# saikumar955078/rl-k8s-scheduler

Measured on AMD Instinct MI355X. Metric: env-steps/sec (node), batched rollout+policy update, 1/2/4/8 GPUs; %HBM BW, higher is better.
Workload: dtype fp32 (split-fp16 MFMA, fp32-accurate); 1 GPU; c4: 131,072 envs/GPU (1,048,576 over 8 GPUs) x 2-cloud table, T=128 rollout + GAE + PPO update (10 epochs x 256 minibatches of 65,536 rows/GPU, FCNet [256,256] tanh); envs_per_gpu=131072, rollout_steps=128, minibatch_per_gpu=65536, epochs=10, global_batch=16777216, global_envs=131072, global_minibatch=65536, sgd_precision=sf16, parallelism=dp1

## Files before the change

include/rlks.h:

```cpp
#ifndef RLKS_H
#define RLKS_H

#include <stdint.h>

#include "rlks_types.h"

#ifdef __cplusplus
extern "C" {
#endif

#define RLKS_OK 0
#define RLKS_ERR_ARG (-1)
#define RLKS_ERR_HIP (-2)
#define RLKS_ERR_UNSUPPORTED (-3)
#define RLKS_ERR_STATE (-4)

const char* rlks_last_error(void);
const char* rlks_version(void);

int rlks_debug_checks(unsigned long long* out);

typedef struct rlks_env rlks_env;

int rlks_env_create(const rlks_env_cfg* cfg, const double* cost_host, const double* lat_host,
// ... 48 lines not shown
             float lam, int T, int N, float* adv_dev, float* vtarg_dev, double* partials_dev,
             void* stream);
int rlks_gae_partials_count(int N);
int rlks_adv_stats(const double* partials_dev, int n_partials, double count, double* sums_dev,
                   void* stream);
int rlks_adv_finalize(const double* sums_dev, float* dyn_dev, void* stream);

#define RLKS_N_TENSORS 12
int rlks_mlp_layout(const rlks_mlp_desc* desc, int64_t* offsets12, int64_t* padded_count,
                    int64_t* real_count);

int rlks_policy_forward(const rlks_mlp_desc* desc, const float* params_dev, const float* obs_dev,
                        int n, float* logits_dev, float* values_dev, void* stream);

typedef struct rlks_rollout_bufs {
  float* obs;
  float* logits;
  float* values;
  int32_t* actions;
  float* logp;
  float* rewards;
  uint8_t* dones;
  float* adv;
  float* vtarg;
  int32_t T;
  int32_t N;
  int32_t global_lanes;
} rlks_rollout_bufs;

int rlks_rollout(rlks_env* env, const rlks_mlp_desc* desc, const float* params_dev,
                 const rlks_rollout_bufs* bufs, int explore, void* stream);
int rlks_policy_forward_ws(const rlks_mlp_desc* desc, const float* params_dev, const float* obs_dev, int n,
                           float* logits_dev, float* values_dev, void* workspace, int64_t ws_bytes, void* stream);
int rlks_gemm_sf16(const rlks_gemm_desc* desc, void* stream);
int rlks_absmax(const float* x, int rows, int cols, int ld, uint32_t* slot, void* stream);
int rlks_rollout_ws(rlks_env* env, const rlks_mlp_desc* desc, const float* params_dev,
                    const rlks_rollout_bufs* bufs, int explore, void* workspace, int64_t ws_bytes,
                    void* stream);

int rlks_minibatch_stride(const rlks_mlp_desc* desc);
int rlks_ppo_gather(const rlks_mlp_desc* desc, const rlks_rollout_bufs* bufs, uint64_t perm_seed,
                    int epoch, int64_t row0, int rows, const float* dyn_dev, float* mb_dev,
                    void* stream);
int rlks_ppo_gather_grouped(const rlks_mlp_desc* desc, const rlks_rollout_bufs* bufs, uint64_t perm_seed,
                            int epoch, int groups, int group0, int64_t row0, int rows, const float* dyn_dev,
                            float* mb_dev, void* stream);
int rlks_packed_stride(const rlks_mlp_desc* desc);
int rlks_ppo_pack(const rlks_mlp_desc* desc, const rlks_rollout_bufs* bufs, float* packed_dev, void* stream);
int rlks_ppo_gather_packed(const rlks_mlp_desc* desc, const float* packed_dev, int T, int N, uint64_t perm_seed,
                           int epoch, int groups, int group0, int64_t row0, int rows, float* mb_dev, void* stream);

int rlks_ppo_workspace_bytes(const rlks_mlp_desc* desc, int rows, int64_t* bytes);
int rlks_debug_sf_handoff(const rlks_mlp_desc* desc, int rows, void* workspace_dev, void** out);
int rlks_debug_wide_bufs(const rlks_mlp_desc* desc, int rows, void* workspace_dev, void** out);
int rlks_ppo_grad(const rlks_mlp_desc* desc, const rlks_ppo_coeffs* coeffs, const float* params_dev,
                  const float* dyn_dev, const float* mb_dev, int rows, float* grad_dev,
                  double* stats_dev, void* workspace_dev, int64_t workspace_bytes, void* stream);

#define RLKS_PHASE_FWD 1
#define RLKS_PHASE_DW2 2
#define RLKS_PHASE_DH1 4
#define RLKS_PHASE_REDUCE 8
#define RLKS_PHASE_ALL 15
#define RLKS_PHASE_FWD_PI 16
#define RLKS_PHASE_FWD_VF 32
#define RLKS_PHASE_PREP 64
#define RLKS_PHASE_F1A 128
#define RLKS_PHASE_F1B 256
int rlks_ppo_grad_phases(const rlks_mlp_desc* desc, const rlks_ppo_coeffs* coeffs, const float* params_dev,
                         const float* dyn_dev, const float* mb_dev, int rows, float* grad_dev, double* stats_dev,
                         void* workspace_dev, int64_t workspace_bytes, int phases, void* stream);

int rlks_ppo_grad_profile(const rlks_mlp_desc* desc, const rlks_ppo_coeffs* coeffs, const float* params_dev,
                          const float* dyn_dev, const float* mb_dev, int rows, float* grad_dev, double* stats_dev,
                          void* workspace_dev, int64_t workspace_bytes, int reps, double* ms_out, void* stream);

int rlks_sf_f1_fused(const rlks_mlp_desc* desc);

int rlks_adam_step(float* params_dev, const float* grad_dev, float* m_dev, float* v_dev, int64_t n,
                   float lr, float beta1, float beta2, float eps, int step, void* stream);
int rlks_ppo_sgd_step(const rlks_mlp_desc* desc, const rlks_ppo_coeffs* coeffs, float* params_dev,
                      const float* dyn_dev, const float* mb_dev, int rows, float* grad_dev, double* stats_dev,
                      float* adam_m_dev, float* adam_v_dev, int64_t n_params, float lr, float beta1, float beta2,
                      float eps, int step, int prev_fused, void* workspace, int64_t ws_bytes, void* stream);

typedef struct rlks_gather_next {
  const float* packed_dev;
  float* mb_dev;
  uint64_t perm_seed;
  int64_t row0;
  int T, N, epoch, groups, group0, rows;
} rlks_gather_next;
int rlks_ppo_sgd_step_next(const rlks_mlp_desc* desc, const rlks_ppo_coeffs* coeffs, float* params_dev,
                           const float* dyn_dev, const float* mb_dev, int rows, float* grad_dev, double* stats_dev,
                           float* adam_m_dev, float* adam_v_dev, int64_t n_params, float lr, float beta1, float beta2,
                           float eps, int step, int prev_fused, const rlks_gather_next* next, void* workspace,
                           int64_t ws_bytes, void* stream);

int rlks_ppo_grad_step(const rlks_mlp_desc* desc, const rlks_ppo_coeffs* coeffs, const float* params_dev,
                       const float* dyn_dev, const float* mb_dev, int rows, float* grad_dev, double* stats_dev,
                       int step, int prev_fused, void* workspace, int64_t ws_bytes, void* stream);
int rlks_ppo_grad_step_next(const rlks_mlp_desc* desc, const rlks_ppo_coeffs* coeffs, const float* params_dev,
                            const float* dyn_dev, const float* mb_dev, int rows, float* grad_dev, double* stats_dev,
                            int step, int prev_fused, const rlks_gather_next* next, void* workspace,
                            int64_t ws_bytes, void* stream);
int rlks_ppo_grad_step_part(const rlks_mlp_desc* desc, const rlks_ppo_coeffs* coeffs, const float* params_dev,
// ... 45 lines not shown
```

rl-k8s-scheduler_amd/csrc/ppo.hip:

```cpp
#include <cmath>

#include "sgd_sf16.h"
#include "wide_mlp.h"

namespace rlks {


struct RedTask {
  const float* part;
  float* out;
  double* out64;
  int64_t pstride;
  int P, len, G, V;
  int blk0;
  int mslot;
  int mbase;
  int kq;
};
constexpr int MAX_TASKS = 20;
struct AdamCo {
  float w1, b2, omb2, step_size, bc2_sqrt, eps;
};
__device__ __forceinline__ float adam_elem(float* __restrict__ p, float* __restrict__ m, float* __restrict__ v,
                                           int64_t i, float gi, const AdamCo& c) {
// ... 904 lines not shown
    RLKS_REQUIRE(bytes && rows > 0 && rows % 256 == 0, RLKS_ERR_ARG,
                 "rlks_ppo_workspace_bytes: split-fp16 rows must be a positive multiple of 256");
    *bytes = sf_ws_layout(d->obs_dim, d->n_actions, rows, nullptr).bytes;
    return RLKS_OK;
  }
  RLKS_REQUIRE(bytes && rows > 0 && rows % GB == 0, RLKS_ERR_ARG,
               "rlks_ppo_workspace_bytes: rows must be a positive multiple of 128");
  *bytes = ws_layout(d->obs_dim, d->n_actions, rows, nullptr).bytes;
  return RLKS_OK;
}

static int nrm_ws_at(const rlks_mlp_desc* d, int rows, void* workspace, int64_t ws_bytes, NrmWs& n) {
  int64_t gb = 0;
  if (int rc = grad_ws_bytes(d, rows, &gb)) return rc;
  gb = (gb + 255) / 256 * 256;
  n = nrm_ws(d, (char*)workspace + gb);
  RLKS_REQUIRE(ws_bytes >= gb + n.bytes, RLKS_ERR_ARG, "grad_clip: workspace too small (rlks_ppo_workspace_bytes)");
  return RLKS_OK;
}

}

extern "C" {

int rlks_ppo_workspace_bytes(const rlks_mlp_desc* d, int rows, int64_t* bytes) {
  if (int rc = grad_ws_bytes(d, rows, bytes)) return rc;
  *bytes = (*bytes + 255) / 256 * 256 + nrm_ws(d, nullptr).bytes;
  return RLKS_OK;
}

int rlks_grad_global_norm(const rlks_mlp_desc* d, const float* grad, int64_t n_params, double* norm_dev,
                          void* workspace, int64_t ws_bytes, void* stream) {
  if (int rc = check_desc(d)) return rc;
  RLKS_REQUIRE(grad && norm_dev && workspace, RLKS_ERR_ARG, "rlks_grad_global_norm: null argument");
  RLKS_REQUIRE(n_params == make_layout(d->obs_dim, d->hidden, d->n_actions).padded, RLKS_ERR_ARG,
               "rlks_grad_global_norm: n_params must be the padded layout size");
  const NrmWs n = nrm_ws(d, (char*)workspace);
  RLKS_REQUIRE(ws_bytes >= n.bytes, RLKS_ERR_ARG, "rlks_grad_global_norm: workspace too small");
  return norm_pass(d, grad, n, 1.f, norm_dev, nullptr, (hipStream_t)stream);
}

int rlks_debug_sf_handoff(const rlks_mlp_desc* d, int rows, void* ws, void** out) {
  if (int rc = check_desc(d)) return rc;
  RLKS_REQUIRE(out && ws && rows > 0 && rows % 256 == 0 && is_sf(d) && !is_wide(d),
               RLKS_ERR_ARG, "rlks_debug_sf_handoff: split-fp16 descriptor, rows % 256 == 0");
  const SfWs w = sf_ws_layout(d->obs_dim, d->n_actions, rows, (char*)ws);
  for (int net = 0; net < 2; ++net) {
    out[net] = w.n[net].dz2s;
    out[2 + net] = w.n[net].tile_edz;
  }
  return RLKS_OK;
}

int rlks_debug_wide_bufs(const rlks_mlp_desc* d, int rows, void* ws, void** out) {
  if (int rc = check_desc(d)) return rc;
  RLKS_REQUIRE(out && ws && rows > 0 && is_wide(d), RLKS_ERR_ARG, "rlks_debug_wide_bufs: wide descriptor");
  const WideWs w = wide_ws_layout(d->obs_dim, d->hidden, d->n_actions, rows, (char*)ws);
  for (int net = 0; net < 2; ++net) {
    out[3 * net] = w.n[net].h2;
    out[3 * net + 1] = w.n[net].out;
    out[3 * net + 2] = w.n[net].dout;
  }
  return RLKS_OK;
}

struct FusedAdam {
  float *p, *m, *v;
  AdamCo co;
  int step, prev_fused;
  bool apply = true;
  int64_t n = 0;
  float clip = 0.f;
};

static int sf_grad(const rlks_mlp_desc* d, const rlks_ppo_coeffs* co, const float* params, const float* dyn,
                   const float* mb, int M, float* grad, double* stats, void* workspace, int64_t ws_bytes, int phases,
                   hipStream_t s, const FusedAdam* fa = nullptr, const NextGather* nx = nullptr, int part = 0,
                   const NrmWs* nrm = nullptr, float clip = 0.f) {
  RLKS_REQUIRE(M > 0 && M % 256 == 0, RLKS_ERR_ARG, "rlks_ppo_grad: split-fp16 rows must be a positive multiple of 256");
  const int D = d->obs_dim, A = d->n_actions, H = HID;
  const SfWs w = sf_ws_layout(D, A, M, (char*)workspace);
  RLKS_REQUIRE(ws_bytes >= w.bytes, RLKS_ERR_ARG, "rlks_ppo_grad: workspace too small");
  const Layout L = make_layout(D, H, A);
  const bool f_pi = phases & (RLKS_PHASE_FWD | RLKS_PHASE_FWD_PI), f_vf = phases & (RLKS_PHASE_FWD | RLKS_PHASE_FWD_VF);
  if (part == 2) phases &= ~(RLKS_PHASE_PREP | RLKS_PHASE_DW2);
  if ((phases & (RLKS_PHASE_FWD | RLKS_PHASE_PREP)) && part != 2) {
    const int parity = fa ? ((fa->step - 1) & 1) : 0;
    if (int rc = sf_prep(d, w, params, s, false, parity, fa && fa->prev_fused, fa ? (unsigned)fa->step : 0u))
      return rc;
  }
  SfArgs a{};
  a.x = mb; a.x_stride = mb_stride(D, A); a.M = M; a.D = D; a.A_pi = A;
  a.tiles_per_split = w.tiles_per_split; a.co = *co; a.dyn = dyn; a.xsp = w.xsp;
  a.products = d->precision == RLKS_PRECISION_F16 ? 1 : 3;
  for (int net = 0; net < 2; ++net) {
    a.n[net] = w.n[net];
    const NetPtrs P = net_ptrs_host(params, L, net);
    a.n[net].b2 = P.b2; a.n[net].w3 = P.w3; a.n[net].b3 = P.b3;
  }
  const int f1ab = phases & (RLKS_PHASE_F1A | RLKS_PHASE_F1B);
  SfF1Form f1;
  if (part != 0) f1 = part == 1 ? SF_F1_A : SF_F1_B;
  else if (f1ab && !(f_pi || f_vf)) f1 = SfF1Form((f1ab & RLKS_PHASE_F1A ? SF_F1_A : 0) | (f1ab & RLKS_PHASE_F1B ? SF_F1_B : 0));
  else f1 = sf_f1_fused(A) ? SF_F1_FUSED : SF_F1_SPLIT;
  if (f_pi || f_vf) {
    if (int rc = launch_sf_f1(a, f_pi ? 0 : 1, (f_pi && f_vf) ? 2 : 1, A, s, f1)) return rc;
// ... 562 lines not shown
```

rl-k8s-scheduler_amd/csrc/sgd_sf16.hip:

```cpp
#include <cmath>
#include <type_traits>

#include "sgd_sf16.h"

namespace rlks {


using h8 = __attribute__((ext_vector_type(8))) _Float16;
using h4 = __attribute__((ext_vector_type(4))) _Float16;
using v4u = __attribute__((ext_vector_type(4))) unsigned;

constexpr int SF_ROWS = 256;
constexpr float SF_H1_SCALE = 16384.f;

__device__ __forceinline__ int sf_perm(int s, int h, int j) { return 16 * s + 8 * (j >> 2) + 4 * h + (j & 3); }
__device__ __forceinline__ int p16(int p) { return 16 * ((p >> 2) & 1) + 4 * (p >> 3) + (p & 3); }

__device__ __forceinline__ f32x16 mma(h8 a, h8 b, f32x16 c) {
  return __builtin_amdgcn_mfma_f32_32x32x16_f16(a, b, c, 0, 0, 0);
}
__device__ __forceinline__ f32x16 mma3(h8 ah, h8 al, h8 bh, h8 bl, f32x16 c) {
  c = mma(al, bh, c);
  c = mma(ah, bl, c);
  return mma(ah, bh, c);
}
template <int P>
__device__ __forceinline__ f32x16 mmaP(h8 ah, h8 al, h8 bh, h8 bl, f32x16 c) {
  if constexpr (P == 1) return __builtin_amdgcn_mfma_f32_32x32x16_f16(ah, bh, c, 0, 0, 0);
  else return mma3(ah, al, bh, bl, c);
}

__device__ __forceinline__ void split1(float x, _Float16& hi, _Float16& lo) {
  hi = (_Float16)x;
  lo = (_Float16)(x - (float)hi);
}
typedef _Float16 hf2 __attribute__((ext_vector_type(2)));
__device__ __forceinline__ void split2(float x0, float x1, unsigned& hi, unsigned& lo) {
  const hf2 h = {(_Float16)x0, (_Float16)x1};
  hi = __builtin_bit_cast(unsigned, h);
  unsigned l;
  asm("v_fma_mixlo_f16 %0, %1, 1.0, -%2 op_sel_hi:[0,0,1]\n\t"
      "v_fma_mixhi_f16 %0, %3, 1.0, -%2 op_sel:[0,0,1] op_sel_hi:[0,0,1]"
      : "=&v"(l)
      : "v"(x0), "v"(hi), "v"(x1));
  lo = l;
}
__device__ __forceinline__ void split8v(const float (&x)[8], h8& hi, h8& lo) {
  v4u h, l;
#pragma unroll
  for (int q = 0; q < 4; ++q) {
    unsigned a, b;
    split2(x[2 * q], x[2 * q + 1], a, b);
    h[q] = a;
    l[q] = b;
// ... 901 lines not shown
        float sum = 0.f;
        const int dq = (d & ~15) + 4 * (((d >> 2) & 3) ^ ((kk >> 1) & 3)) + (d & 3);
#pragma unroll
        for (int ww = 0; ww < W; ++ww) sum += sEp[jj * SLOT + (ww * 16 + kk) * 16 * DT + dq];
        if (d < ND - 1) N.part_w1[((size_t)blk * HID + k) * (ND - 1) + d] = sum;
        else N.part_b1[(size_t)blk * HID + k] = sum;
      }
      if (kt < 15) __syncthreads();
    }
  }
  FB_STAMP(5);
}

template <int KD, int ND, int W, int P>
__global__ __launch_bounds__(64 * W) __attribute__((amdgpu_waves_per_eu(4, 4))) void k_sf_bwd(SfArgs g) {
  const int2 ng = f1_net_group<W, true>(g);
  if (ng.x + g.net0 == 0) f1b_body<0, KD, ND, W, P>(g, ng.y);
  else f1b_body<1, KD, ND, W, P>(g, ng.y);
}

template <int A_, int KD, int W>
constexpr bool f1_w1_kept() {
  return W * (A_ - 1 > 1 ? A_ - 1 : 1) * HID * 4 + W * (A_ + 4) * 4 <= 4 * H16 * 2;
}
template <int A_, int KD, int W>
constexpr int f1_lds_bytes() {
  constexpr int ab = f1a_lds_bytes<A_, KD, W>() > f1b_lds_bytes<KD>() ? f1a_lds_bytes<A_, KD, W>() : f1b_lds_bytes<KD>();
  constexpr int ep = KD == 16 ? F1_EP_BYTES : 0;
  return ab > ep ? ab : ep;
}
template <int A_>
constexpr bool f1_x_kept() { return A_ <= 4; }
template <int A_, int KD, int W, int P>
__global__ __launch_bounds__(64 * W) __attribute__((amdgpu_waves_per_eu(4, 4))) void k_sf_f1(SfArgs g) {
  const int2 ng = f1_net_group<W, (A_ <= 4)>(g);
  SfArgs g2 = g;
  constexpr int XOFF = f1_x_kept<A_>() ? f1_lds_bytes<A_, KD, W>() : -1;
  DzFrag dz0;
  if (ng.x + g.net0 == 0) {
    const int2 e = f1a_body<A_, 0, KD, W, P, XOFF>(g, ng.y, &dz0);
    __syncthreads();
    asm volatile("" : "+s"(g2.x));
    f1b_body<0, KD, 3 * A_ + 1, W, P, true, f1_w1_kept<A_, KD, W>(), XOFF>(g2, ng.y, e.x, e.y, &dz0);
  } else {
    const int2 e = f1a_body<1, 1, KD, W, P, XOFF>(g, ng.y, &dz0);
    __syncthreads();
    asm volatile("" : "+s"(g2.x));
    f1b_body<1, KD, 3 * A_ + 1, W, P, true, f1_w1_kept<1, KD, W>(), XOFF>(g2, ng.y, e.x, e.y, &dz0);
  }
}

#ifdef RLKS_STAMPS
__device__ unsigned long long g_f2_stamps[2][128][16][6];
#endif
constexpr int F2_THREADS = 512;
constexpr int F2_AROW = HID + 32;
constexpr int F2_APLANE = 32 * F2_AROW;
constexpr int F2R_ABUF = 2 * F2_APLANE;
constexpr int F2_MAX_TILES = 2 * 256;

template <int KD, int P>
__global__ __launch_bounds__(F2_THREADS) void k_sf_dw2r(SfArgs g) {
  const SfNet& N = g.n[blockIdx.y];
  extern __shared__ __attribute__((aligned(16))) float lds[];
  _Float16* sm = reinterpret_cast<_Float16*>(lds);
  const int tid = threadIdx.x, l = tid & 63, w = __builtin_amdgcn_readfirstlane(tid >> 6);
  const int c = l & 15, gq = l >> 4, r = l & 31, h = l >> 5;
  int t0 = blockIdx.x * g.tiles_per_split, t1 = t0 + g.tiles_per_split;
  if (!dcheck(t1 <= g.M / 32, DC_SGD_TILE, t1)) t0 = t1 = 0;
  const int nk = t1 - t0;

  int* sEx = reinterpret_cast<int*>(sm + 2 * F2R_ABUF);
  int* sEd = sEx + F2_MAX_TILES;
  int emin = 120;
  for (int i = tid; i < 2 * nk; i += F2_THREADS) {
    sEx[i] = N.tile_ex[2 * t0 + i];
    const int e = N.tile_edz[2 * t0 + i];
    sEd[i] = e;
    emin = min(emin, e);
  }
  __shared__ float s_emin[F2_THREADS / 64];
  emin = (int)-wave_max((float)-emin);
  if (l == 0) s_emin[w] = (float)emin;
  __syncthreads();
#pragma unroll
  for (int i = 0; i < F2_THREADS / 64; ++i) emin = min(emin, (int)s_emin[i]);
  const int E = __builtin_amdgcn_readfirstlane(emin);
  const float ssgn = tile_sign(blockIdx.x);
  const float unscale = ssgn * pow2(-14 - E);

  const int aq = (4 * ((l >> 4) & 1) + (l & 3)) ^ (2 * h);
  const int bbase = (4 * h + ((l & 15) >> 2)) * F2_AROW + 4 * aq;
  const int bbase8 = (4 * h + ((l & 15) >> 2) + 8) * F2_AROW + 4 * (aq ^ 4);
  f32x16 acc[8];
#pragma unroll
  for (int j = 0; j < 8; ++j)
#pragma unroll
    for (int q = 0; q < 16; ++q) acc[j][q] = 0.f;
  auto mfma_chunk = [&](const _Float16* b, const h8 (&hh)[2], const h8 (&hl)[2]) {
#pragma unroll
    for (int s = 0; s < 2; ++s)
#pragma unroll
      for (int ob = 0; ob < 8; ++ob) {
        const _Float16* pb = b + bbase + s * 16 * F2_AROW + 32 * ob;
        const _Float16* pb8 = b + bbase8 + s * 16 * F2_AROW + 32 * ob;
        const h4 a0 = tr_read(pb), a1 = tr_read(pb8);
        const h4 c0 = tr_read(pb + F2_APLANE), c1 = tr_read(pb8 + F2_APLANE);
        const h8 bh = __builtin_shufflevector(a0, a1, 0, 1, 2, 3, 4, 5, 6, 7);
        const h8 bl = __builtin_shufflevector(c0, c1, 0, 1, 2, 3, 4, 5, 6, 7);
        acc[ob] = mmaP<P>(hh[s], hl[s], bh, bl, acc[ob]);
      }
  };

  const __amdgpu_buffer_rsrc_t dz_rsrc = __builtin_amdgcn_make_buffer_rsrc(N.dz2s, (short)0, 0x7fffffff, 0x00020000);
  const int dz_lane = 2 * (w * 1024 + l * 8);
  h8 dp[4];
  auto load_dz = [&](int t) {
#pragma unroll
    for (int i = 0; i < 4; ++i)
      dp[i] = __builtin_bit_cast(h8, __builtin_amdgcn_raw_buffer_load_b128(
                                         dz_rsrc, dz_lane, t * (32 * HID * 4) + (i >> 1) * (16 * HID * 4) + (i & 1) * 1024, 0));
  };
  float db2[8] = {};
  auto store_dz = [&](_Float16* img, float s0, float s1) {
#pragma unroll
    for (int i = 0; i < 4; ++i) {
      const float sc = (i >> 1) ? s1 : s0;
#pragma unroll
      for (int j = 0; j < 8; ++j) db2[j] = fmaf((float)dp[i][j], sc, db2[j]);
      const int off = (i & 1) * F2_APLANE + (16 * (i >> 1) + c) * F2_AROW + 32 * w;
      const int sw = 2 * ((c >> 2) & 3);
      *reinterpret_cast<h4*>(img + off + 4 * (gq ^ sw)) = __builtin_shufflevector(dp[i], dp[i], 0, 1, 2, 3);
      *reinterpret_cast<h4*>(img + off + 4 * ((gq + 4) ^ sw)) = __builtin_shufflevector(dp[i], dp[i], 4, 5, 6, 7);
    }
  };

  constexpr int KB = KD / 8;
  const int kh = 32 * w + r;
  h4 wh[KB], wl[KB];
  auto load_w1 = [&]() {
#pragma unroll
    for (int kb = 0; kb < KB; ++kb) {
      wh[kb] = *reinterpret_cast<const h4*>(N.w1h + kh * KD + 8 * kb + 4 * h);
      wl[kb] = *reinterpret_cast<const h4*>(N.w1l + kh * KD + 8 * kb + 4 * h);
    }
  };
  if constexpr (KB <= 2) load_w1();
  const float inv_w1 = N.sc[1];
  h4 xrh[KB], xrl[KB];
  int2 xe, de;
  const __amdgpu_buffer_rsrc_t x_rsrc = __builtin_amdgcn_make_buffer_rsrc(g.xsp, (short)0, 0x7fffffff, 0x00020000);
  const int xlo = 2 * g.M * KD;
  auto load_x = [&](int t) {
    xe = *reinterpret_cast<const int2*>(sEx + 2 * (t - t0));
    de = *reinterpret_cast<const int2*>(sEd + 2 * (t - t0));
#pragma unroll
    for (int kb = 0; kb < KB; ++kb) {
      const int off = 2 * (r * KD + 8 * kb + 4 * h);
      xrh[kb] = __builtin_bit_cast(h4, __builtin_amdgcn_raw_buffer_load_b64(x_rsrc, off, 2 * t * 32 * KD, 0));
      xrl[kb] = __builtin_bit_cast(h4, __builtin_amdgcn_raw_buffer_load_b64(x_rsrc, off + xlo, 2 * t * 32 * KD, 0));
    }
  };
  auto make_h1 = [&](h8 (&hh)[2], h8 (&hl)[2]) {
    if constexpr (KB > 2) load_w1();
    f32x16 z;
#pragma unroll
    for (int q = 0; q < 16; ++q) z[q] = 0.f;
#pragma unroll
    for (int kb = 0; kb < KB; ++kb) {
      if constexpr (P != 1) {
        z = __builtin_amdgcn_mfma_f32_32x32x8f16(xrl[kb], wh[kb], z, 0, 0, 0);
        z = __builtin_amdgcn_mfma_f32_32x32x8f16(xrh[kb], wl[kb], z, 0, 0, 0);
      }
      z = __builtin_amdgcn_mfma_f32_32x32x8f16(xrh[kb], wh[kb], z, 0, 0, 0);
    }
    const float kz0 = inv_w1 * pow2(-xe.x) * SF_2LOG2E, kz1 = -inv_w1 * pow2(-xe.y) * SF_2LOG2E;
    const float hs0 = ssgn * pow2(14 + E - de.x), hs1 = -ssgn * pow2(14 + E - de.y);
#pragma unroll
    for (int s = 0; s < 2; ++s) {
      const float hs = s ? hs1 : hs0, kz = s ? kz1 : kz0;
      float x[8];
#pragma unroll
      for (int j = 0; j < 8; ++j) x[j] = fmaf(-2.f * hs, tanh_r(z[8 * s + j] * kz), hs);
      split8v(x, hh[s], hl[s]);
    }
  };
  auto barrier = [&]() {
    __builtin_amdgcn_sched_barrier(0);
    asm volatile("s_waitcnt lgkmcnt(0)" ::: "memory");
    __builtin_amdgcn_s_barrier();
    asm volatile("" ::: "memory");
    __builtin_amdgcn_sched_barrier(0);
  };

  h8 hh[2], hl[2];
  if (nk > 0) {
    load_dz(t0);
    load_x(t0);
    store_dz(sm, pow2(-de.x), -pow2(-de.y));
    make_h1(hh, hl);
    load_x(min(t0 + 1, t1 - 1));
    load_dz(min(t0 + 1, t1 - 1));
  }
  __syncthreads();
  if (KD == 16 && w >= 4) {
    for (int ci = 0; ci < nk; ++ci) {
      const bool counted = ci + 1 < nk;
      const float s0 = counted ? pow2(-de.x) : 0.f, s1 = counted ? -pow2(-de.y) : 0.f;
      h8 nh[2], nl[2];
      store_dz(sm + ((ci + 1) & 1) * F2R_ABUF, s0, s1);
      make_h1(nh, nl);
      load_x(min(t0 + ci + 2, t1 - 1));
      __builtin_amdgcn_sched_barrier(0);
      load_dz(min(t0 + ci + 2, t1 - 1));
      mfma_chunk(sm + (ci & 1) * F2R_ABUF, hh, hl);
      barrier();
#pragma unroll
      for (int s = 0; s < 2; ++s) {
        hh[s] = nh[s];
        hl[s] = nl[s];
      }
    }
  } else
  for (int ci = 0; ci < nk; ++ci) {
    mfma_chunk(sm + (ci & 1) * F2R_ABUF, hh, hl);
    const bool counted = ci + 1 < nk;
    const float s0 = counted ? pow2(-de.x) : 0.f, s1 = counted ? -pow2(-de.y) : 0.f;
    h8 nh[2], nl[2];
    store_dz(sm + ((ci + 1) & 1) * F2R_ABUF, s0, s1);
    make_h1(nh, nl);
    load_x(min(t0 + ci + 2, t1 - 1));
    __builtin_amdgcn_sched_barrier(0);
    load_dz(min(t0 + ci + 2, t1 - 1));
    barrier();
#pragma unroll
    for (int s = 0; s < 2; ++s) {
      hh[s] = nh[s];
      hl[s] = nl[s];
    }
  }

  float* out = N.part_w2 + (size_t)blockIdx.x * SF_W2_PSTRIDE;
#pragma unroll
  for (int ob = 0; ob < 8; ++ob)
#pragma unroll
    for (int t = 0; t < 4; ++t) {
      const v4f v = {acc[ob][4 * t] * unscale, acc[ob][4 * t + 1] * unscale, acc[ob][4 * t + 2] * unscale,
                     acc[ob][4 * t + 3] * unscale};
      *reinterpret_cast<v4f*>(out + ((size_t)(8 * w + 2 * t + h) * HID + 32 * ob + r) * 4) = v;
    }
#pragma unroll
  for (int j = 0; j < 8; ++j) db2[j] = row_sum16(db2[j]);
  if (c == 0)
#pragma unroll
    for (int j = 0; j < 8; ++j) N.part_b2[(size_t)blockIdx.x * HID + 32 * w + 16 * (j >> 2) + 4 * gq + (j & 3)] = db2[j];
}


__device__ __forceinline__ int x_frag_rows(const float* __restrict__ x, int row, int D, int g, h8& xh, h8& xl) {
  const float* xr = x + (size_t)row * D;
  float xv[8];
#pragma unroll
  for (int j = 0; j < 8; ++j) xv[j] = xa_elem(xr, 8 * g + j, D);
  float xm = 0.f;
#pragma unroll
  for (int j = 0; j < 8; ++j) xm = fmaxf(xm, fabsf(xv[j]));
  const int ex = sf_exp(wave_max(xm));
  split8(xv, 0, pow2(ex), xh, xl);
  return ex;
}

template <int A_, int KD, int W>
constexpr int fwd16_lds_bytes() {
  return 4 * H16 * 2 + 2 * HID * KD * 2 + (HID + A_ * HID) * 4;
}

template <int A_, int NET, int KD, int W>
__device__ __forceinline__ void fwd16_body(const SfFwdArgs& g) {
  constexpr int NTHR = 64 * W;
  const SfNet& N = g.n[NET];
  extern __shared__ __attribute__((aligned(16))) float lds[];
  _Float16* sCh = reinterpret_cast<_Float16*>(lds);
  _Float16* sW1 = sCh + 4 * H16;
  float* sB2 = lds + (4 * H16 * 2 + 2 * HID * KD * 2) / 4;
  float* sW3 = sB2 + HID;

  const int tid = threadIdx.x, l = tid & 63, w = __builtin_amdgcn_readfirstlane(tid >> 6), c = l & 15, gq = l >> 4;
  const int row0 = (blockIdx.x * W + w) * 16;
  const int row = min(row0 + c, g.M - 1);

  hc_dma<W>(N.w2ph, N.w2pl, 0, 0, sCh, w, l);
  for (int i = tid; i < HID; i += NTHR) sB2[i] = N.b2[i] * SF_2LOG2E;
  for (int i = tid; i < A_ * HID; i += NTHR) sW3[i] = N.w3[i];
  w1_stage<KD, NTHR>(N, sW1, tid);
  h8 xh, xl;
  const int ex = x_frag_rows(g.x, row, g.D, gq, xh, xl);
  const float k_z1 = N.sc[1] * pow2(-ex) * SF_2LOG2E;
  vm_drain();
  __syncthreads();

  f4 acc[16];
#pragma unroll
  for (int nt = 0; nt < 16; ++nt) acc[nt] = f4zero();
  h8 bh, bl;
  for (int t = 0; t < 8; ++t) {
#pragma unroll
    for (int ph = 0; ph < 2; ++ph) {
      const int st = 2 * t + ph;
// ... 176 lines not shown
```

rl-k8s-scheduler_amd/rlks/_lib.py:

```python
from __future__ import annotations

import ctypes as C
import os
from pathlib import Path

PKG_DIR = Path(__file__).resolve().parent
LIB_PATH = Path(os.environ.get("RLKS_LIB", PKG_DIR / "librlks.so"))

RLKS_NOISE_PHILOX = 0
RLKS_NOISE_MT19937 = 1
RLKS_N_TENSORS = 12
RLKS_DYN_SIZE = 8
RLKS_DYN_ADV_MEAN, RLKS_DYN_ADV_INVSTD, RLKS_DYN_KL_COEFF, RLKS_DYN_INV_COUNT = 0, 1, 2, 3
RLKS_STAT_SIZE = 8
RLKS_PHASE_FWD, RLKS_PHASE_DW2, RLKS_PHASE_DH1, RLKS_PHASE_REDUCE, RLKS_PHASE_ALL = 1, 2, 4, 8, 15
RLKS_PHASE_FWD_PI, RLKS_PHASE_FWD_VF, RLKS_PHASE_PREP, RLKS_PHASE_F1A, RLKS_PHASE_F1B = 16, 32, 64, 128, 256
RLKS_PRECISION_FP32, RLKS_PRECISION_SF16, RLKS_PRECISION_WIDE, RLKS_PRECISION_F16 = 0, 1, 2, 3
RLKS_STAT_POLICY_LOSS, RLKS_STAT_VF_LOSS, RLKS_STAT_KL, RLKS_STAT_ENTROPY, RLKS_STAT_ROWS = 0, 1, 2, 3, 4
RLKS_STAT_GRAD_GNORM = 5
RLKS_EPLOG_CAP = 128
(RLKS_RM_ROWS, RLKS_RM_REWARD_SUM, RLKS_RM_REWARD_MIN, RLKS_RM_REWARD_MAX, RLKS_RM_DONES, RLKS_RM_VALUE_SUM,
 RLKS_RM_VTARG_SUM, RLKS_RM_VTARG_SQ, RLKS_RM_RESID_SUM, RLKS_RM_RESID_SQ, RLKS_RM_FIXED) = range(11)
(RLKS_RULE_ROUND_ROBIN, RLKS_RULE_CHEAPEST, RLKS_RULE_MYOPIC, RLKS_RULE_LEAST_LOADED, RLKS_RULE_MYOPIC_WITH_ROOM,
 RLKS_RULE_RANDOM) = range(6)
# ... 18 lines not shown


class GemmDesc(C.Structure):
    _fields_ = [("a", C.c_void_p), ("b", C.c_void_p), ("c", C.c_void_p), ("bias", C.c_void_p), ("aux", C.c_void_p),
                ("m", C.c_int32), ("n", C.c_int32), ("k", C.c_int32), ("lda", C.c_int32), ("ldb", C.c_int32),
                ("ldc", C.c_int32), ("ldaux", C.c_int32), ("trans_a", C.c_int32), ("trans_b", C.c_int32),
                ("epilogue", C.c_int32), ("accumulate", C.c_int32), ("reserved", C.c_int32),
                ("a_max", C.c_void_p), ("b_max", C.c_void_p), ("c_max", C.c_void_p)]


RLKS_GEMM_STORE, RLKS_GEMM_TANH_BIAS, RLKS_GEMM_BIAS, RLKS_GEMM_DTANH = 0, 1, 2, 3


class MlpDesc(C.Structure):
    _fields_ = [("obs_dim", C.c_int32), ("hidden", C.c_int32), ("n_actions", C.c_int32), ("precision", C.c_int32)]


class PpoCoeffs(C.Structure):
    _fields_ = [("clip_param", C.c_float), ("vf_clip_param", C.c_float), ("vf_loss_coeff", C.c_float),
                ("entropy_coeff", C.c_float)]


class RolloutBufs(C.Structure):
    _fields_ = [("obs", C.c_void_p), ("logits", C.c_void_p), ("values", C.c_void_p), ("actions", C.c_void_p),
                ("logp", C.c_void_p), ("rewards", C.c_void_p), ("dones", C.c_void_p), ("adv", C.c_void_p),
                ("vtarg", C.c_void_p), ("T", C.c_int32), ("N", C.c_int32), ("global_lanes", C.c_int32)]


class GatherNext(C.Structure):
    _fields_ = [("packed", C.c_void_p), ("mb", C.c_void_p), ("perm_seed", C.c_uint64), ("row0", C.c_int64),
                ("T", C.c_int32), ("N", C.c_int32), ("epoch", C.c_int32), ("groups", C.c_int32),
                ("group0", C.c_int32), ("rows", C.c_int32)]


_P = C.c_void_p
_I = C.c_int
_I64 = C.c_int64
_F = C.c_float

SIGNATURES = {
    "rlks_last_error": [],
    "rlks_version": [],
    "rlks_env_create": [C.POINTER(EnvCfg), _P, _P, C.POINTER(_P)],
    "rlks_env_create_ext": [C.POINTER(EnvCfg), _P, _P, _P, _P, _P, _I, C.POINTER(_P)],
    "rlks_env_destroy": [_P],
    "rlks_env_node_state": [_P, _P, _P, _P, _P],
    "rlks_env_counters": [_P, _I, _P, _P],
    "rlks_env_config": [_P, C.POINTER(EnvCfg)],
    "rlks_env_seed": [_P, _P, _P, _P, _I, _P],
    "rlks_env_mt_discard": [_P, _P, _P, _P],
    "rlks_env_mt_words": [_P, C.c_int, _P, C.c_int, _P],
    "rlks_debug_checks": [_P],
    "rlks_debug_sf_handoff": [C.POINTER(MlpDesc), _I, _P, _P],
    "rlks_debug_wide_bufs": [C.POINTER(MlpDesc), _I, _P, _P],
    "rlks_sample_categorical": [_P, C.c_int, C.c_int, _P, C.c_ulonglong, C.c_int, _P, _P, _P],
    "rlks_env_reset": [_P, _P, _P, _P],
    "rlks_env_step": [_P, _P, _P, _P, _P, _P, _P, _P, _P, _P, _P],
    "rlks_env_sample_step": [_P, _P, _I, _P, _P, _P, _P, _P, _P],
    "rlks_env_rule_actions": [_P, _I, _P, _P, _P],
    "rlks_env_episode_stats": [_P, _P, _I, _P],
    "rlks_env_lane_state": [_P, _P, _P, _P],
    "rlks_env_episode_log": [_P, _P, _P, _P, _I, _P],
    "rlks_env_state_bytes": [_P, C.POINTER(_I64)],
    "rlks_env_save_state": [_P, _P, _P],
    "rlks_env_load_state": [_P, _P, _P],
    "rlks_philox4x32_10": [_P, _P, _P, _I, _P],
    "rlks_mt_random": [_P, _I, _P, _I, _P],
    "rlks_gae": [_P, _P, _P, _F, _F, _I, _I, _P, _P, _P, _P],
    "rlks_gae_partials_count": [_I],
    "rlks_adv_stats": [_P, _I, C.c_double, _P, _P],
    "rlks_adv_finalize": [_P, _P, _P],
    "rlks_mlp_layout": [C.POINTER(MlpDesc), C.POINTER(_I64), C.POINTER(_I64), C.POINTER(_I64)],
    "rlks_policy_forward": [C.POINTER(MlpDesc), _P, _P, _I, _P, _P, _P],
    "rlks_rollout": [_P, C.POINTER(MlpDesc), _P, C.POINTER(RolloutBufs), _I, _P],
    "rlks_gemm_sf16": [C.POINTER(GemmDesc), _P],
    "rlks_absmax": [_P, _I, _I, _I, _P, _P],
    "rlks_policy_forward_ws": [C.POINTER(MlpDesc), _P, _P, _I, _P, _P, _P, _I64, _P],
    "rlks_rollout_ws": [_P, C.POINTER(MlpDesc), _P, C.POINTER(RolloutBufs), _I, _P, _I64, _P],
    "rlks_minibatch_stride": [C.POINTER(MlpDesc)],
    "rlks_ppo_gather": [C.POINTER(MlpDesc), C.POINTER(RolloutBufs), C.c_uint64, _I, _I64, _I, _P, _P, _P],
    "rlks_ppo_gather_grouped": [C.POINTER(MlpDesc), C.POINTER(RolloutBufs), C.c_uint64, _I, _I, _I, _I64, _I, _P,
                                _P, _P],
    "rlks_packed_stride": [C.POINTER(MlpDesc)],
    "rlks_ppo_pack": [C.POINTER(MlpDesc), C.POINTER(RolloutBufs), _P, _P],
    "rlks_ppo_gather_packed": [C.POINTER(MlpDesc), _P, _I, _I, C.c_uint64, _I, _I, _I, _I64, _I, _P, _P],
    "rlks_ppo_workspace_bytes": [C.POINTER(MlpDesc), _I, C.POINTER(_I64)],
    "rlks_ppo_grad": [C.POINTER(MlpDesc), C.POINTER(PpoCoeffs), _P, _P, _P, _I, _P, _P, _P, _I64, _P],
    "rlks_ppo_grad_phases": [C.POINTER(MlpDesc), C.POINTER(PpoCoeffs), _P, _P, _P, _I, _P, _P, _P, _I64, _I, _P],
    "rlks_ppo_grad_profile": [C.POINTER(MlpDesc), C.POINTER(PpoCoeffs), _P, _P, _P, _I, _P, _P, _P, _I64, _I, _P, _P],
    "rlks_sf_f1_fused": [C.POINTER(MlpDesc)],
    "rlks_adam_step": [_P, _P, _P, _P, _I64, _F, _F, _F, _F, _I, _P],
    "rlks_ppo_sgd_step": [C.POINTER(MlpDesc), C.POINTER(PpoCoeffs), _P, _P, _P, _I, _P, _P, _P, _P, _I64, _F, _F, _F,
                          _F, _I, _I, _P, _I64, _P],
    "rlks_ppo_sgd_step_next": [C.POINTER(MlpDesc), C.POINTER(PpoCoeffs), _P, _P, _P, _I, _P, _P, _P, _P, _I64, _F,
                               _F, _F, _F, _I, _I, C.POINTER(GatherNext), _P, _I64, _P],
    "rlks_ppo_grad_step": [C.POINTER(MlpDesc), C.POINTER(PpoCoeffs), _P, _P, _P, _I, _P, _P, _I, _I, _P, _I64, _P],
    "rlks_ppo_grad_step_next": [C.POINTER(MlpDesc), C.POINTER(PpoCoeffs), _P, _P, _P, _I, _P, _P, _I, _I,
                                C.POINTER(GatherNext), _P, _I64, _P],
    "rlks_ppo_grad_step_part": [C.POINTER(MlpDesc), C.POINTER(PpoCoeffs), _P, _P, _P, _I, _P, _P, _I, _I, _I,
                                C.POINTER(GatherNext), _P, _I64, _P],
    "rlks_ppo_adam_apply": [C.POINTER(MlpDesc), _P, _P, _P, _P, _I64, _F, _F, _F, _F, _I, _P, _I64, _I, _P],
    "rlks_grad_global_norm": [C.POINTER(MlpDesc), _P, _I64, _P, _P, _I64, _P],
    "rlks_ppo_sgd_step_clip": [C.POINTER(MlpDesc), C.POINTER(PpoCoeffs), _P, _P, _P, _I, _P, _P, _P, _P, _I64, _F,
                               _F, _F, _F, _I, _I, _F, C.POINTER(GatherNext), _P, _I64, _P],
    "rlks_ppo_adam_apply_clip": [C.POINTER(MlpDesc), _P, _P, _P, _P, _I64, _F, _F, _F, _F, _I, _F, _P, _P, _I64, _I,
                                 _P],
# ... 74 lines not shown
```

Measured before the change: 31.41 million env-steps/s.

## Stream dz tiles into LDS via global_load_lds and pipeline transposed fragment reads

The dW2 reduction kernel no longer loads dz2 tiles into registers and writes them to a swizzled LDS image. It now DMAs them directly into a pre-laid-out LDS buffer with global_load_lds, one tile ahead. The MFMA inner loop uses explicit ds_read_b64_tr_b16 fragment reads with a one-step lookahead and counted lgkmcnt waits, and db2 sums are read back from LDS. W1 loading is hoisted out of make_h1 for all KD, timing stamps are added under RLKS_STAMPS, and a debug layout query is exposed. This cuts VGPR pressure and LDS store traffic, but it relies on a precise global dz2s layout and on hand-tuned waitcnt.

Result: no change. 31.57 million env-steps/s (median of 6 runs) (+0.5%).

```diff
diff --git a/include/rlks.h b/include/rlks.h
--- a/include/rlks.h
+++ b/include/rlks.h
@@ -124,6 +124,7 @@
 
 int rlks_ppo_workspace_bytes(const rlks_mlp_desc* desc, int rows, int64_t* bytes);
 int rlks_debug_sf_handoff(const rlks_mlp_desc* desc, int rows, void* workspace_dev, void** out);
+int rlks_debug_sf_f2_layout(const rlks_mlp_desc* desc, int rows, int* out);
 int rlks_debug_wide_bufs(const rlks_mlp_desc* desc, int rows, void* workspace_dev, void** out);
 int rlks_ppo_grad(const rlks_mlp_desc* desc, const rlks_ppo_coeffs* coeffs, const float* params_dev,
                   const float* dyn_dev, const float* mb_dev, int rows, float* grad_dev,
diff --git a/rl-k8s-scheduler_amd/csrc/ppo.hip b/rl-k8s-scheduler_amd/csrc/ppo.hip
--- a/rl-k8s-scheduler_amd/csrc/ppo.hip
+++ b/rl-k8s-scheduler_amd/csrc/ppo.hip
@@ -980,6 +980,16 @@
   return RLKS_OK;
 }
 
+int rlks_debug_sf_f2_layout(const rlks_mlp_desc* d, int rows, int* out) {
+  if (int rc = check_desc(d)) return rc;
+  RLKS_REQUIRE(out && rows > 0 && rows % 256 == 0 && is_sf(d) && !is_wide(d), RLKS_ERR_ARG,
+               "rlks_debug_sf_f2_layout: split-fp16 descriptor, rows % 256 == 0");
+  const SfWs w = sf_ws_layout(d->obs_dim, d->n_actions, rows, nullptr);
+  out[0] = w.splits;
+  out[1] = w.tiles_per_split;
+  return RLKS_OK;
+}
+
 int rlks_debug_wide_bufs(const rlks_mlp_desc* d, int rows, void* ws, void** out) {
   if (int rc = check_desc(d)) return rc;
   RLKS_REQUIRE(out && ws && rows > 0 && is_wide(d), RLKS_ERR_ARG, "rlks_debug_wide_bufs: wide descriptor");
diff --git a/rl-k8s-scheduler_amd/csrc/sgd_sf16.hip b/rl-k8s-scheduler_amd/csrc/sgd_sf16.hip
--- a/rl-k8s-scheduler_amd/csrc/sgd_sf16.hip
+++ b/rl-k8s-scheduler_amd/csrc/sgd_sf16.hip
@@ -1,5 +1,6 @@
 #include <cmath>
 #include <type_traits>
+#include <utility>
 
 #include "sgd_sf16.h"
 
@@ -1007,12 +1008,71 @@
 
 #ifdef RLKS_STAMPS
 __device__ unsigned long long g_f2_stamps[2][128][16][6];
+#define F2_STAMP_INIT()                                                \
+  unsigned long long f2_ph[5] = {}, f2_t = __builtin_amdgcn_s_memtime(); \
+  const unsigned long long f2_start = f2_t
+#define F2_STAMP(i)                                                  \
+  {                                                                  \
+    const unsigned long long f2_now = __builtin_amdgcn_s_memtime();  \
+    f2_ph[i] += f2_now - f2_t;                                       \
+    f2_t = f2_now;                                                   \
+  }
+#define F2_STAMP_FLUSH()                                                                   \
+  if (l == 0 && blockIdx.x < 128) {                                                        \
+    for (int i = 0; i < 5; ++i) g_f2_stamps[blockIdx.y][blockIdx.x][w][i] = f2_ph[i];      \
+    g_f2_stamps[blockIdx.y][blockIdx.x][w][5] = f2_start;                                  \
+  }
+#else
+#define F2_STAMP_INIT()
+#define F2_STAMP(i)
+#define F2_STAMP_FLUSH()
 #endif
 constexpr int F2_THREADS = 512;
-constexpr int F2_AROW = HID + 32;
-constexpr int F2_APLANE = 32 * F2_AROW;
-constexpr int F2R_ABUF = 2 * F2_APLANE;
+constexpr int F2_BLK = 64 * 8;
+constexpr int F2_NSTEP = 2 * F2_BLK;
+constexpr int F2_TILE = 8 * F2_NSTEP;
+constexpr int F2R_ABUF = 2 * F2_TILE;
+constexpr int F2_AHEAD = 1;
 constexpr int F2_MAX_TILES = 2 * 256;
+__device__ __forceinline__ int f2_dma_piece(int d) { return 16 * (d & 3) + (d >> 2); }
+__device__ __forceinline__ int f2_tr_slot(int l) { return 4 * (4 * (l >> 5) + ((l & 15) >> 2)) + (l & 3); }
+__device__ __forceinline__ int f2_own_slot(int l) { return 4 * (l & 15) + (l >> 4); }
+
+template <int P>
+struct F2Frag {
+  using v2u = __attribute__((ext_vector_type(2))) unsigned;
+  static constexpr int READS = P == 1 ? 2 : 4;
+  v2u a0, a1, c0, c1;
+  template <int OFF>
+  __device__ __forceinline__ void read(unsigned addr) {
+    asm volatile("ds_read_b64_tr_b16 %0, %1 offset:%2" : "=v"(a0) : "v"(addr), "n"(OFF) : "memory");
+    asm volatile("ds_read_b64_tr_b16 %0, %1 offset:%2" : "=v"(a1) : "v"(addr), "n"(OFF + 512) : "memory");
+    if constexpr (P != 1) {
+      asm volatile("ds_read_b64_tr_b16 %0, %1 offset:%2" : "=v"(c0) : "v"(addr), "n"(OFF + 2 * F2_BLK) : "memory");
+      asm volatile("ds_read_b64_tr_b16 %0, %1 offset:%2" : "=v"(c1) : "v"(addr), "n"(OFF + 2 * F2_BLK + 512) : "memory");
+    }
+  }
+  template <int N>
+  __device__ __forceinline__ void landed() {
+    if constexpr (P != 1) asm volatile("s_waitcnt lgkmcnt(%4)" : "+v"(a0), "+v"(a1), "+v"(c0), "+v"(c1) : "n"(N) : "memory");
+    else asm volatile("s_waitcnt lgkmcnt(%2)" : "+v"(a0), "+v"(a1) : "n"(N) : "memory");
+  }
+  __device__ __forceinline__ h8 hi() const {
+    return __builtin_bit_cast(h8, __builtin_shufflevector(a0, a1, 0, 1, 2, 3));
+  }
+  __device__ __forceinline__ h8 lo() const {
+    if constexpr (P != 1) return __builtin_bit_cast(h8, __builtin_shufflevector(c0, c1, 0, 1, 2, 3));
+    else return hi();
+  }
+};
+template <class F, int... I>
+__device__ __forceinline__ void f2_static_for_seq(F&& f, std::integer_sequence<int, I...>) {
+  (f(std::integral_constant<int, I>{}), ...);
+}
+template <int N, class F>
+__device__ __forceinline__ void f2_static_for(F&& f) {
+  f2_static_for_seq(f, std::make_integer_sequence<int, N>{});
+}
 
 template <int KD, int P>
 __global__ __launch_bounds__(F2_THREADS) void k_sf_dw2r(SfArgs g) {
@@ -1024,6 +1084,7 @@
   int t0 = blockIdx.x * g.tiles_per_split, t1 = t0 + g.tiles_per_split;
   if (!dcheck(t1 <= g.M / 32, DC_SGD_TILE, t1)) t0 = t1 = 0;
   const int nk = t1 - t0;
+  F2_STAMP_INIT();
 
   int* sEx = reinterpret_cast<int*>(sm + 2 * F2R_ABUF);
   int* sEd = sEx + F2_MAX_TILES;
@@ -1044,49 +1105,49 @@
   const float ssgn = tile_sign(blockIdx.x);
   const float unscale = ssgn * pow2(-14 - E);
 
-  const int aq = (4 * ((l >> 4) & 1) + (l & 3)) ^ (2 * h);
-  const int bbase = (4 * h + ((l & 15) >> 2)) * F2_AROW + 4 * aq;
-  const int bbase8 = (4 * h + ((l & 15) >> 2) + 8) * F2_AROW + 4 * (aq ^ 4);
+  const int bbase = f2_tr_slot(l) * 8 + 4 * ((l >> 4) & 1);
   f32x16 acc[8];
 #pragma unroll
   for (int j = 0; j < 8; ++j)
 #pragma unroll
     for (int q = 0; q < 16; ++q) acc[j][q] = 0.f;
   auto mfma_chunk = [&](const _Float16* b, const h8 (&hh)[2], const h8 (&hl)[2]) {
-#pragma unroll
-    for (int s = 0; s < 2; ++s)
-#pragma unroll
-      for (int ob = 0; ob < 8; ++ob) {
-        const _Float16* pb = b + bbase + s * 16 * F2_AROW + 32 * ob;
-        const _Float16* pb8 = b + bbase8 + s * 16 * F2_AROW + 32 * ob;
-        const h4 a0 = tr_read(pb), a1 = tr_read(pb8);
-        const h4 c0 = tr_read(pb + F2_APLANE), c1 = tr_read(pb8 + F2_APLANE);
-        const h8 bh = __builtin_shufflevector(a0, a1, 0, 1, 2, 3, 4, 5, 6, 7);
-        const h8 bl = __builtin_shufflevector(c0, c1, 0, 1, 2, 3, 4, 5, 6, 7);
-        acc[ob] = mmaP<P>(hh[s], hl[s], bh, bl, acc[ob]);
-      }
+    const unsigned pb = (unsigned)(size_t)(__attribute__((address_space(3))) const _Float16*)(b + bbase);
+    constexpr int AH = F2_AHEAD;
+    F2Frag<P> f[AH + 1];
+    f2_static_for<AH>([&](auto ic) {
+      constexpr int n = decltype(ic)::value;
+      f[n].template read<2 * ((n >> 3) * F2_TILE + (n & 7) * F2_NSTEP)>(pb);
+    });
+    f2_static_for<16>([&](auto ic) {
+      constexpr int i = decltype(ic)::value, n = i + AH;
+      if constexpr (n < 16) f[n % (AH + 1)].template read<2 * ((n >> 3) * F2_TILE + (n & 7) * F2_NSTEP)>(pb);
+      __builtin_amdgcn_sched_barrier(0);
+      f[i % (AH + 1)].template landed<F2Frag<P>::READS * (15 - i < AH ? 15 - i : AH)>();
+      acc[i & 7] = mmaP<P>(hh[i >> 3], hl[i >> 3], f[i % (AH + 1)].hi(), f[i % (AH + 1)].lo(), acc[i & 7]);
+      __builtin_amdgcn_sched_barrier(0);
+    });
   };
 
-  const __amdgpu_buffer_rsrc_t dz_rsrc = __builtin_amdgcn_make_buffer_rsrc(N.dz2s, (short)0, 0x7fffffff, 0x00020000);
-  const int dz_lane = 2 * (w * 1024 + l * 8);
-  h8 dp[4];
-  auto load_dz = [&](int t) {
-#pragma unroll
-    for (int i = 0; i < 4; ++i)
-      dp[i] = __builtin_bit_cast(h8, __builtin_amdgcn_raw_buffer_load_b128(
-                                         dz_rsrc, dz_lane, t * (32 * HID * 4) + (i >> 1) * (16 * HID * 4) + (i & 1) * 1024, 0));
+  const char* dz_src = reinterpret_cast<const char*>(N.dz2s) + (unsigned)(2 * w * F2_NSTEP + 16 * f2_dma_piece(l));
+  auto dma_dz = [&](int t, _Float16* img) {
+#pragma unroll
+    for (int i = 0; i < 4; ++i) {
+      const int blk = (i >> 1) * F2_TILE + (i & 1) * F2_BLK;
+      __builtin_amdgcn_global_load_lds(dz_src + (size_t)t * (2 * F2R_ABUF) + 2 * blk,
+                                       (__attribute__((address_space(3))) void*)(img + w * F2_NSTEP + blk), 16, 0, 0);
+    }
   };
   float db2[8] = {};
-  auto store_dz = [&](_Float16* img, float s0, float s1) {
+  auto sum_db2 = [&](const _Float16* img, int ci) {
+    const int2 e = *reinterpret_cast<const int2*>(sEd + 2 * ci);
+    const float s0 = pow2(-e.x), s1 = -pow2(-e.y);
 #pragma unroll
     for (int i = 0; i < 4; ++i) {
       const float sc = (i >> 1) ? s1 : s0;
-#pragma unroll
-      for (int j = 0; j < 8; ++j) db2[j] = fmaf((float)dp[i][j], sc, db2[j]);
-      const int off = (i & 1) * F2_APLANE + (16 * (i >> 1) + c) * F2_AROW + 32 * w;
-      const int sw = 2 * ((c >> 2) & 3);
-      *reinterpret_cast<h4*>(img + off + 4 * (gq ^ sw)) = __builtin_shufflevector(dp[i], dp[i], 0, 1, 2, 3);
-      *reinterpret_cast<h4*>(img + off + 4 * ((gq + 4) ^ sw)) = __builtin_shufflevector(dp[i], dp[i], 4, 5, 6, 7);
+      const h8 dp = *reinterpret_cast<const h8*>(img + w * F2_NSTEP + (i >> 1) * F2_TILE + (i & 1) * F2_BLK + 8 * f2_own_slot(l));
+#pragma unroll
+      for (int j = 0; j < 8; ++j) db2[j] = fmaf((float)dp[j], sc, db2[j]);
     }
   };
 
@@ -1100,15 +1161,17 @@
       wl[kb] = *reinterpret_cast<const h4*>(N.w1l + kh * KD + 8 * kb + 4 * h);
     }
   };
-  if constexpr (KB <= 2) load_w1();
+  load_w1();
   const float inv_w1 = N.sc[1];
   h4 xrh[KB], xrl[KB];
   int2 xe, de;
   const __amdgpu_buffer_rsrc_t x_rsrc = __builtin_amdgcn_make_buffer_rsrc(g.xsp, (short)0, 0x7fffffff, 0x00020000);
   const int xlo = 2 * g.M * KD;
-  auto load_x = [&](int t) {
+  auto load_e = [&](int t) {
     xe = *reinterpret_cast<const int2*>(sEx + 2 * (t - t0));
     de = *reinterpret_cast<const int2*>(sEd + 2 * (t - t0));
+  };
+  auto load_x = [&](int t) {
 #pragma unroll
     for (int kb = 0; kb < KB; ++kb) {
       const int off = 2 * (r * KD + 8 * kb + 4 * h);
@@ -1117,7 +1180,6 @@
     }
   };
   auto make_h1 = [&](h8 (&hh)[2], h8 (&hl)[2]) {
-    if constexpr (KB > 2) load_w1();
     f32x16 z;
 #pragma unroll
     for (int q = 0; q < 16; ++q) z[q] = 0.f;
@@ -1142,7 +1204,7 @@
   };
   auto barrier = [&]() {
     __builtin_amdgcn_sched_barrier(0);
-    asm volatile("s_waitcnt lgkmcnt(0)" ::: "memory");
+    asm volatile("s_waitcnt vmcnt(%0) lgkmcnt(0)" ::"n"(2 * KB) : "memory");
     __builtin_amdgcn_s_barrier();
     asm volatile("" ::: "memory");
     __builtin_amdgcn_sched_barrier(0);
@@ -1150,26 +1212,31 @@
 
   h8 hh[2], hl[2];
   if (nk > 0) {
-    load_dz(t0);
+    load_e(t0);
+    dma_dz(t0, sm);
     load_x(t0);
-    store_dz(sm, pow2(-de.x), -pow2(-de.y));
     make_h1(hh, hl);
+    load_e(min(t0 + 1, t1 - 1));
     load_x(min(t0 + 1, t1 - 1));
-    load_dz(min(t0 + 1, t1 - 1));
-  }
+  }
+  vm_drain();
   __syncthreads();
+  F2_STAMP(0);
   if (KD == 16 && w >= 4) {
     for (int ci = 0; ci < nk; ++ci) {
-      const bool counted = ci + 1 < nk;
-      const float s0 = counted ? pow2(-de.x) : 0.f, s1 = counted ? -pow2(-de.y) : 0.f;
       h8 nh[2], nl[2];
-      store_dz(sm + ((ci + 1) & 1) * F2R_ABUF, s0, s1);
+      sum_db2(sm + (ci & 1) * F2R_ABUF, ci);
       make_h1(nh, nl);
+      load_e(min(t0 + ci + 2, t1 - 1));
+      __builtin_amdgcn_sched_barrier(0);
+      dma_dz(min(t0 + ci + 1, t1 - 1), sm + ((ci + 1) & 1) * F2R_ABUF);
       load_x(min(t0 + ci + 2, t1 - 1));
       __builtin_amdgcn_sched_barrier(0);
-      load_dz(min(t0 + ci + 2, t1 - 1));
+      F2_STAMP(2);
       mfma_chunk(sm + (ci & 1) * F2R_ABUF, hh, hl);
+      F2_STAMP(1);
       barrier();
+      F2_STAMP(3);
 #pragma unroll
       for (int s = 0; s < 2; ++s) {
         hh[s] = nh[s];
@@ -1178,16 +1245,18 @@
     }
   } else
   for (int ci = 0; ci < nk; ++ci) {
+    dma_dz(min(t0 + ci + 1, t1 - 1), sm + ((ci + 1) & 1) * F2R_ABUF);
+    __builtin_amdgcn_sched_barrier(0);
     mfma_chunk(sm + (ci & 1) * F2R_ABUF, hh, hl);
-    const bool counted = ci + 1 < nk;
-    const float s0 = counted ? pow2(-de.x) : 0.f, s1 = counted ? -pow2(-de.y) : 0.f;
+    F2_STAMP(1);
     h8 nh[2], nl[2];
-    store_dz(sm + ((ci + 1) & 1) * F2R_ABUF, s0, s1);
+    sum_db2(sm + (ci & 1) * F2R_ABUF, ci);
     make_h1(nh, nl);
+    load_e(min(t0 + ci + 2, t1 - 1));
     load_x(min(t0 + ci + 2, t1 - 1));
-    __builtin_amdgcn_sched_barrier(0);
-    load_dz(min(t0 + ci + 2, t1 - 1));
+    F2_STAMP(2);
     barrier();
+    F2_STAMP(3);
 #pragma unroll
     for (int s = 0; s < 2; ++s) {
       hh[s] = nh[s];
@@ -1209,6 +1278,8 @@
   if (c == 0)
 #pragma unroll
     for (int j = 0; j < 8; ++j) N.part_b2[(size_t)blockIdx.x * HID + 32 * w + 16 * (j >> 2) + 4 * gq + (j & 3)] = db2[j];
+  F2_STAMP(4);
+  F2_STAMP_FLUSH();
 }
 
 
diff --git a/rl-k8s-scheduler_amd/rlks/_lib.py b/rl-k8s-scheduler_amd/rlks/_lib.py
--- a/rl-k8s-scheduler_amd/rlks/_lib.py
+++ b/rl-k8s-scheduler_amd/rlks/_lib.py
@@ -94,6 +94,7 @@
     "rlks_env_mt_words": [_P, C.c_int, _P, C.c_int, _P],
     "rlks_debug_checks": [_P],
     "rlks_debug_sf_handoff": [C.POINTER(MlpDesc), _I, _P, _P],
+    "rlks_debug_sf_f2_layout": [C.POINTER(MlpDesc), _I, _P],
     "rlks_debug_wide_bufs": [C.POINTER(MlpDesc), _I, _P, _P],
     "rlks_sample_categorical": [_P, C.c_int, C.c_int, _P, C.c_ulonglong, C.c_int, _P, _P, _P],
     "rlks_env_reset": [_P, _P, _P, _P],
```
